# microsoft/DiskANN

Hardware: NVIDIA H100
Metric: QPS @ recall@10>=0.95, 1Mx128 f32 L2 (Vamana R=64 greedy search, batch 10K) (higher is better)
Workload: dtype f32

## Files before the change

diskann_b200/csrc/dab_common.cuh:

```cuda
#pragma once

#include <cuda_fp16.h>
#include <cuda_runtime.h>

#include <atomic>
#include <cstdarg>
#include <cstdint>
#include <cstdio>
#include <cstring>

#include "../../include/diskann_b200.h"

struct dab_index;

namespace dab {

constexpr uint32_t kNoId = 0xFFFFFFFFu;

char* error_buffer();
int fail(int code, const char* fmt, ...);
extern std::atomic<uint64_t> g_launches;
void comm_release(struct ::dab_index* idx);
void tc_release(struct ::dab_index* idx);
void search_slots_release(struct ::dab_index* idx);

#define DAB_CUDA(expr)                                                                        \
    do {                                                                                      \
        cudaError_t _e = (expr);                                                              \
        if (_e != cudaSuccess)                                                                \
            return ::dab::fail(_e == cudaErrorMemoryAllocation ? DAB_ERR_OUT_OF_MEMORY         \
                                                               : DAB_ERR_CUDA,               \
                               "%s failed: %s (%s:%d)", #expr, cudaGetErrorString(_e),        \
                               __FILE__, __LINE__);                                           \
    } while (0)

#define DAB_LAUNCHED() (::dab::g_launches.fetch_add(1, std::memory_order_relaxed))

inline size_t elem_size(int dtype) {
    switch (dtype) {
        case DAB_F32: return 4;
        case DAB_F16: return 2;
        default: return 1;
    }
}
inline size_t round_up(size_t x, size_t m) { return (x + m - 1) / m * m; }

struct Scratch {
    void* p = nullptr;
    size_t bytes = 0;
    bool pinned_host = false;
    int reserve(size_t n);
    void release();
};

struct Tuning {
    int test_visited_log2 = 0;
    bool test_pq_global_lut = false;
    void load();
};

}

struct dab_index {
    int dtype = 0, metric = 0;
    uint32_t dim = 0;
    uint64_t n_points = 0;
    uint32_t n_start = 0;
    uint32_t max_degree = 0;
    int device = 0;
    int sm_count = 132;

    cudaStream_t stream = nullptr;
    cudaStream_t own_stream = nullptr;

    uint8_t* d_vectors = nullptr;
    size_t row_stride = 0;
    uint32_t* d_adj = nullptr;
    uint32_t adj_stride = 0;
    bool vectors_ready = false, graph_ready = false;

    float* d_pivots = nullptr;
    uint32_t* d_offsets = nullptr;
    uint8_t* d_codes = nullptr;
    uint32_t pq_chunks = 0, pq_centers = 0;
    uint32_t pq_uniform_len = 0;
    bool pq_codes_ready = false;
    int sq_nbits = 0;
    float sq_scale = 0.0f, sq_shift_square_norm = 0.0f, sq_mean_norm = 0.0f;
    float* d_sq_shift = nullptr;
    uint8_t* d_sq_codes = nullptr;
    float* d_sq_comp = nullptr;
    uint32_t sq_row_bytes = 0, sq_stride = 0;
    bool sq_codes_ready = false;

    dab::Scratch s_queries, s_ids, s_out, s_out2, s_tables, s_counters, s_stats;
    dab::Scratch h_stage;
    dab::Scratch h_counters;
    void* slots[DAB_MAX_SLOTS] = {};

    uint32_t hint_l = 0, hint_beam = 0, hint_visited = 0;
    uint32_t pq_hint_l = 0, pq_hint_beam = 0, pq_hint_visited = 0; int pq_hint_mode = 0;
    uint32_t v3_overflow_l = 0, v3_overflow_beam = 0;
    float v3_overflow_frac = 0.0f;
    void* l2_window_ptr = nullptr;
    size_t l2_window_bytes = 0;
    cudaStream_t l2_window_stream = nullptr;

    uint64_t rec_truncated = 0;
    dab::Tuning tune;

    void* d_tc_base = nullptr;
    void* d_tc_coef = nullptr;
    uint64_t tc_version = 0, vectors_version = 1;

    void* nccl_comm = nullptr;
    int nccl_rank = 0, nccl_ranks = 0;

    uint64_t n_total() const { return n_points + n_start; }
};
```

diskann_b200/csrc/search_kernel.cu:

```cuda
#include "dab_common.cuh"
#include "distance_device.cuh"
#include "search_v2.cuh"
#include "search_v3.cuh"

#include <algorithm>
#include <cstdlib>

namespace dab {

constexpr int kSearchWarps = 4;
constexpr uint32_t kEmpty = 0xFFFFFFFFu;
constexpr uint32_t kVisitedFlag = 0x80000000u;
constexpr int kRowsInFlight = 4;

struct SearchParams {
    const uint8_t* vectors;
    size_t row_stride;
    const uint32_t* adj;
    uint32_t adj_stride;
    uint64_t n_points;
    uint32_t n_start;
    uint32_t dim;
    uint32_t max_degree;
    const void* queries;
// ... 185 lines not shown
                    else if (c0 == 64) word = w2;
                    else word = c0 + lane < p.adj_stride ? __ldg(row + c0 + lane) : kEmpty;
                    const uint32_t j = c0 + lane;
                    const bool valid = j >= 1 && j <= deg;
                    bool inserted = false;
                    if (valid) inserted = visited_insert(table, p.hcap_log2, word);
                    const bool isnew = inserted && word < n_total;
                    const unsigned mi = __ballot_sync(kFull, inserted);
                    const unsigned mn = __ballot_sync(kFull, isnew);
                    if (isnew) cid[ncand + __popc(mn & ((1u << lane) - 1u))] = word;
                    ncand += __popc(mn);
                    nvisited += __popc(mi);
                }
                if (nvisited + p.max_degree + 32 > hlimit) {
                    overflow = true;
                    break;
                }
            }
            if (overflow) break;
            __syncwarp();

            for (uint32_t c0 = 0; c0 < ncand; c0 += TEAMS * U) {
                float r[U];
                uint32_t cc[U];
                if constexpr (IS_INT) {
                    const uint8_t* rows[U];
#pragma unroll
                    for (int u = 0; u < U; ++u) {
                        cc[u] = c0 + u;
                        const uint32_t id = cid[min(cc[u], ncand - 1)];
                        rows[u] = p.vectors + (size_t)id * p.row_stride;
                    }
                    warp_int_multi<SIGNED, KIND, U>(qb, rows, dim, lane, qq, r);
                } else {
                    const TD* rows[U];
#pragma unroll
                    for (int u = 0; u < U; ++u) {
                        cc[u] = c0 + u * TEAMS + team;
                        const uint32_t id = cid[min(cc[u], ncand - 1)];
                        rows[u] = reinterpret_cast<const TD*>(p.vectors + (size_t)id * p.row_stride);
                    }
                    team_float_multi<NA, KIND, U>(qf, rows, dim, slot, r);
                }
#pragma unroll
                for (int u = 0; u < U; ++u)
                    if (slot == 0 && cc[u] < ncand) cd[cc[u]] = post_op<POST>(r[u]);
            }
            __syncwarp();

            for (uint32_t c = 0; c < ncand; ++c) queue_insert(qd, qi, p.cap, size, cursor, cid[c], cd[c], lane);
            cmps += ncand;
            hops += nb;
        }

        if (overflow) {
            if (lane == 0) {
                uint32_t o = atomicAdd(p.counters + 1, 1u);
                p.overflow_list[o] = qidx;
            }
            continue;
        }

        {
            const uint32_t n = min(p.cap, size);
            uint32_t count = 0;
            for (uint32_t b = 0; b < n && count < p.k; b += 32) {
                const uint32_t i = b + lane;
                uint32_t id = i < n ? (qi[i] & ~kVisitedFlag) : kEmpty;
                const bool keep = i < n && id < p.n_points;
                const unsigned m = __ballot_sync(kFull, keep);
                const uint32_t pos = count + __popc(m & ((1u << lane) - 1u));
                if (keep && pos < p.k) {
                    p.out_ids[(size_t)qidx * p.k + pos] = id;
                    p.out_dists[(size_t)qidx * p.k + pos] = qd[i];
                }
                count += __popc(m);
            }
            count = min(count, p.k);
            for (uint32_t i = count + lane; i < p.k; i += 32) {
                p.out_ids[(size_t)qidx * p.k + i] = kEmpty;
                p.out_dists[(size_t)qidx * p.k + i] = __int_as_float(0x7F800000);
            }
            if (lane == 0) {
                atomicMax(p.counters + 2, nvisited);
                if (p.out_counts) p.out_counts[qidx] = count;
                if (p.out_cmps) p.out_cmps[qidx] = cmps;
                if (p.out_hops) p.out_hops[qidx] = hops;
                if (p.rec_counts) {
                    p.rec_counts[qidx] = min(nrec, p.rec_cap);
                    if (nrec > p.rec_cap) atomicAdd(p.counters + 3, 1u);
                }
            }
        }
    }
}


constexpr int kV2WarpsHost = kV2Warps;

static uint32_t next_pow2_log2(uint64_t v) {
    uint32_t l = 0;
    while ((1ull << l) < v) ++l;
    return l;
}

static void pin_tables_in_l2(dab_index* idx, size_t bytes) {
    void* want = bytes ? idx->s_tables.p : nullptr;
    if (idx->l2_window_ptr == want && idx->l2_window_bytes == bytes && (bytes == 0 || idx->l2_window_stream == idx->stream)) return;
    cudaStreamAttrValue attr;
    memset(&attr, 0, sizeof(attr));
    if (bytes == 0) {
        attr.accessPolicyWindow.num_bytes = 0;
        attr.accessPolicyWindow.hitProp = cudaAccessPropertyNormal;
        attr.accessPolicyWindow.missProp = cudaAccessPropertyNormal;
        if (cudaStreamSetAttribute(idx->l2_window_stream, cudaStreamAttributeAccessPolicyWindow, &attr) != cudaSuccess) cudaGetLastError();
        idx->l2_window_ptr = nullptr;
        idx->l2_window_bytes = 0;
        return;
    }
    int max_persist = 0, max_window = 0;
    cudaDeviceGetAttribute(&max_persist, cudaDevAttrMaxPersistingL2CacheSize, idx->device);
    cudaDeviceGetAttribute(&max_window, cudaDevAttrMaxAccessPolicyWindowSize, idx->device);
    if (max_persist <= 0 || max_window <= 0) return;
    cudaDeviceSetLimit(cudaLimitPersistingL2CacheSize, (size_t)max_persist);
    attr.accessPolicyWindow.base_ptr = idx->s_tables.p;
    attr.accessPolicyWindow.num_bytes = std::min<size_t>(bytes, (size_t)max_window);
    attr.accessPolicyWindow.hitRatio = bytes <= (size_t)max_persist ? 1.0f : (float)((double)max_persist / (double)bytes);
    attr.accessPolicyWindow.hitProp = cudaAccessPropertyPersisting;
    attr.accessPolicyWindow.missProp = cudaAccessPropertyStreaming;
    if (cudaStreamSetAttribute(idx->stream, cudaStreamAttributeAccessPolicyWindow, &attr) != cudaSuccess) {
        cudaGetLastError();
        return;
    }
    idx->l2_window_ptr = idx->s_tables.p;
    idx->l2_window_bytes = bytes;
    idx->l2_window_stream = idx->stream;
}

template <typename K>
static int launch_one(K kern, const dab_index* idx, SearchParams& p, size_t smem_block, int& grid_out) {
    DAB_CUDA(cudaFuncSetAttribute(kern, cudaFuncAttributeMaxDynamicSharedMemorySize, (int)smem_block));
    int per_sm = 0;
    DAB_CUDA(cudaOccupancyMaxActiveBlocksPerMultiprocessor(&per_sm, kern, kSearchWarps * 32, smem_block));
    if (per_sm < 1) return fail(DAB_ERR_INVALID_ARGUMENT, "search kernel does not fit: %zu B shared memory per CTA", smem_block);
    grid_out = per_sm * idx->sm_count;
    return DAB_OK;
}

struct SearchJob {
    dab_index* idx = nullptr;
    cudaStream_t stream = nullptr;
    Scratch* tables = nullptr;
    Scratch* counters = nullptr;
    uint32_t* h_counters = nullptr;
    bool use_window = false;
    bool full_grid = false;

    uint32_t nq = 0, l_search = 0, beam = 0;
    bool recording = false;
    SearchParams p;
    SearchParamsV2 p2;
    SearchParamsV3 p3;
    void (*kern)(const SearchParams) = nullptr;
    size_t smem_block = 0;
    int grid = 0;
    bool use_v2 = false;
    V2Launch v2;
    V3Launch v3;
    uint64_t slots = 0;
    int stage = 1;
    int pass = 0;
    Scratch retry_list;
    uint32_t *d_counters = nullptr, *d_overflow = nullptr;

    int prepare(const void* d_queries, const uint32_t* d_query_rows, uint32_t nq_, uint32_t k, uint32_t l_search_, uint32_t beam_,
                uint32_t* d_ids, float* d_dists, uint32_t* d_counts, uint32_t* d_cmps, uint32_t* d_hops, uint32_t* rec_ids,
                float* rec_dists, uint32_t* rec_counts, uint32_t rec_cap);
    int launch();
    int finish();
    ~SearchJob() { retry_list.release(); }
};

int SearchJob::prepare(const void* d_queries, const uint32_t* d_query_rows, uint32_t nq_, uint32_t k, uint32_t l_search_,
                       uint32_t beam_, uint32_t* d_ids, float* d_dists, uint32_t* d_counts, uint32_t* d_cmps, uint32_t* d_hops,
                       uint32_t* rec_ids, float* rec_dists, uint32_t* rec_counts, uint32_t rec_cap) {
    nq = nq_, l_search = l_search_, beam = beam_;
    recording = rec_ids != nullptr;
    const bool is_int = idx->dtype == DAB_I8 || idx->dtype == DAB_U8;
    const MetricPlan plan = plan_for(idx->metric, is_int);

    memset(&p, 0, sizeof(p));
    p.vectors = idx->d_vectors;
    p.row_stride = idx->row_stride;
    p.adj = idx->d_adj;
    p.adj_stride = idx->adj_stride;
    p.n_points = idx->n_points;
    p.n_start = idx->n_start;
    p.dim = idx->dim;
    p.max_degree = idx->max_degree;
    p.queries = d_queries;
    p.query_rows = d_query_rows;
    p.k = k;
    p.cap = l_search + idx->n_start;
    p.beam = beam;
    p.out_ids = d_ids;
    p.out_dists = d_dists;
    p.out_counts = d_counts;
    p.out_cmps = d_cmps;
    p.out_hops = d_hops;
    p.rec_ids = rec_ids;
    p.rec_dists = rec_dists;
    p.rec_counts = rec_counts;
    p.rec_cap = rec_cap;

    size_t off = 0;
    const size_t qbytes = is_int ? round_up(idx->dim, 4) : (size_t)idx->dim * 4;
    off = round_up(qbytes, 16);
    p.off_qd = (uint32_t)off;
    off += round_up((size_t)p.cap * 4, 16);
    p.off_qi = (uint32_t)off;
    off += round_up((size_t)p.cap * 4, 16);
    const size_t ncand_max = (size_t)beam * idx->max_degree;
    p.off_cid = (uint32_t)off;
    off += round_up(ncand_max * 4, 16);
    p.off_cd = (uint32_t)off;
    off += round_up(ncand_max * 4, 16);
    p.off_beam = (uint32_t)off;
    off += round_up((size_t)beam * 4, 16);
    p.warp_smem = (uint32_t)off;
    smem_block = off * kSearchWarps;
    if (smem_block > 220 * 1024)
        return fail(DAB_ERR_INVALID_ARGUMENT, "search: L=%u, beam=%u, dim=%u need %zu B shared memory per CTA (> 220 KiB)",
                    l_search, beam, idx->dim, smem_block);

    int rc = DAB_OK;
#define PICK(TD, NA, K, P, II, SG)                               \
    do {                                                         \
        kern = search_kernel<TD, NA, K, P, II, SG>;              \
        rc = launch_one(kern, idx, p, smem_block, grid);         \
    } while (0)
#define PICK_FLOAT(TD)                                                                   \
    do {                                                                                 \
        if (plan.kind == KIND_L2) PICK(TD, 4, KIND_L2, POST_ID, false, false);            \
        else if (plan.kind == KIND_IP && plan.post == POST_NEG) PICK(TD, 4, KIND_IP, POST_NEG, false, false); \
        else if (plan.kind == KIND_IP) PICK(TD, 4, KIND_IP, POST_ONE_MINUS, false, false); \
        else PICK(TD, 2, KIND_COS, POST_ONE_MINUS, false, false);                         \
    } while (0)
#define PICK_INT(SG)                                                                     \
    do {                                                                                 \
        if (plan.kind == KIND_L2) PICK(uint8_t, 4, KIND_L2, POST_ID, true, SG);           \
        else if (plan.kind == KIND_IP) PICK(uint8_t, 4, KIND_IP, POST_NEG, true, SG);     \
        else PICK(uint8_t, 4, KIND_COS, POST_ONE_MINUS, true, SG);                        \
    } while (0)
    switch (idx->dtype) {
        case DAB_F32: PICK_FLOAT(float); break;
        case DAB_F16: PICK_FLOAT(__half); break;
        case DAB_I8: PICK_INT(true); break;
        default: PICK_INT(false); break;
    }
#undef PICK
#undef PICK_FLOAT
#undef PICK_INT
    if (rc) return rc;

    memset(&p2, 0, sizeof(p2));
    use_v2 = v2_prepare(idx, l_search, beam, full_grid, p2, v2) == 0;
    if (use_v2) {
        p2.vectors = p.vectors;
        p2.row_stride = p.row_stride;
        p2.adj = p.adj;
        p2.adj_stride = p.adj_stride;
        p2.n_points = p.n_points;
        p2.n_start = p.n_start;
        p2.dim = p.dim;
        p2.max_degree = p.max_degree;
        p2.queries = p.queries;
        p2.query_rows = p.query_rows;
        p2.k = p.k;
        p2.cap = p.cap;
        p2.beam = p.beam;
        p2.out_ids = p.out_ids;
        p2.out_dists = p.out_dists;
        p2.out_counts = p.out_counts;
        p2.out_cmps = p.out_cmps;
        p2.out_hops = p.out_hops;
        p2.rec_ids = p.rec_ids;
        p2.rec_dists = p.rec_dists;
        p2.rec_counts = p.rec_counts;
        p2.rec_cap = p.rec_cap;
        grid = v2.grid;
    }

    double est = 1.1 * idx->max_degree * 1.3 * (double)l_search;
    const bool hinted = idx->hint_visited > 0 && l_search <= idx->hint_l && beam <= idx->hint_beam;
    if (hinted) {
        const double seen = ((double)idx->hint_visited * 1.15 + idx->max_degree) / (use_v2 ? 0.875 : 0.75) + 8.0;
        if (seen < est) est = seen;
    }
    if (est > (double)idx->n_total() * 1.34) est = (double)idx->n_total() * 1.34;
    slots = std::max<uint64_t>(256, (uint64_t)est + 1);
    if (idx->tune.test_visited_log2) slots = 1ull << idx->tune.test_visited_log2;

    if ((rc = counters->reserve(16 + (size_t)nq * 4))) return rc;
    d_counters = (uint32_t*)counters->p;
    d_overflow = d_counters + 4;
    p.counters = d_counters;
    p.overflow_list = d_overflow;
    p.n_work = nq;
    p.query_list = nullptr;
    p2.counters = d_counters;
    p2.overflow_list = d_overflow;

    stage = 1;
    pass = 0;
    uint32_t need = 0;
    if (hinted) need = (uint32_t)std::min<double>((double)idx->hint_visited * 1.15, 4.0e9);
    if (idx->tune.test_visited_log2) need = (1u << idx->tune.test_visited_log2) / 2;
    const bool skip = idx->v3_overflow_l == l_search && idx->v3_overflow_beam == beam && idx->v3_overflow_frac > 0.25f;
    memset(&p3, 0, sizeof(p3));
    if (!skip && v3_prepare(idx, l_search, beam, need, p3, v3) == 0) {
        stage = 0;
        p3.vectors = p.vectors, p3.row_stride = p.row_stride, p3.adj = p.adj, p3.adj_stride = p.adj_stride;
        p3.n_points = p.n_points, p3.n_start = p.n_start, p3.dim = p.dim, p3.max_degree = p.max_degree;
        p3.queries = p.queries, p3.query_rows = p.query_rows, p3.query_list = nullptr, p3.n_work = nq;
        p3.k = p.k, p3.cap = p.cap, p3.beam = p.beam;
        p3.out_ids = p.out_ids, p3.out_dists = p.out_dists, p3.out_counts = p.out_counts;
        p3.out_cmps = p.out_cmps, p3.out_hops = p.out_hops;
        p3.rec_ids = p.rec_ids, p3.rec_dists = p.rec_dists, p3.rec_counts = p.rec_counts, p3.rec_cap = p.rec_cap;
        p3.counters = d_counters, p3.overflow_list = d_overflow;
    }
    return DAB_OK;
}

int SearchJob::launch() {
    DAB_CUDA(cudaMemsetAsync(d_counters, 0, 16, stream));
    if (stage == 0) {
        const uint64_t max_workers = (uint64_t)v3.grid * kV3Warps;
        const uint64_t rounds = (nq + max_workers - 1) / max_workers;
        const uint64_t need_warps = (nq + rounds - 1) / rounds;
        const int launch_grid = (int)((need_warps + kV3Warps - 1) / kV3Warps);
        v3.kern<<<launch_grid, kV3Warps * 32, v3.smem_block, stream>>>(p3);
    } else {
        const uint32_t warps = (uint32_t)grid * (use_v2 ? kV2WarpsHost : kSearchWarps);
        const uint32_t hlog = std::max<uint32_t>(use_v2 ? 8 : 10, next_pow2_log2(slots));
        const uint32_t n_buckets = (uint32_t)((slots + 7) / 8);
        const size_t words_per_warp = use_v2 ? (size_t)n_buckets * 8 : ((size_t)1 << hlog);
        int rc;
        if ((rc = tables->reserve((size_t)warps * words_per_warp * 4))) return rc;
        p.tables = (uint32_t*)tables->p;
        p.hcap_log2 = hlog;
        if (use_window) pin_tables_in_l2(idx, use_v2 ? 0 : (size_t)warps * words_per_warp * 4);
        if (use_v2) {
            const uint64_t max_warps = (uint64_t)grid * kV2WarpsHost;
            const uint64_t rounds = (p.n_work + max_warps - 1) / max_warps;
            const uint64_t need = (p.n_work + rounds - 1) / rounds;
            int launch_grid = (int)((need + kV2WarpsHost - 1) / kV2WarpsHost);
            if (full_grid) launch_grid = (int)std::min<uint64_t>((uint64_t)grid, ((uint64_t)p.n_work + kV2WarpsHost - 1) / kV2WarpsHost);
            p2.tables = p.tables;
            p2.n_buckets = n_buckets;
            p2.query_list = p.query_list;
            p2.n_work = p.n_work;
            v2.kern<<<launch_grid, kV2WarpsHost * 32, v2.smem_block, stream>>>(p2);
        } else {
            const int launch_grid = (int)std::min<uint64_t>((uint64_t)grid, ((uint64_t)p.n_work + kSearchWarps - 1) / kSearchWarps);
            kern<<<launch_grid, kSearchWarps * 32, smem_block, stream>>>(p);
        }
    }
    DAB_LAUNCHED();
    DAB_CUDA(cudaGetLastError());
    DAB_CUDA(cudaMemcpyAsync(h_counters, d_counters, 16, cudaMemcpyDeviceToHost, stream));
    return DAB_OK;
}

int SearchJob::finish() {
    for (;;) {
        DAB_CUDA(cudaStreamSynchronize(stream));
        idx->rec_truncated += h_counters[3];
        const uint32_t n_over = h_counters[1];
        if (!recording) {
            if (l_search != idx->hint_l || beam != idx->hint_beam) {
                idx->hint_l = l_search;
                idx->hint_beam = beam;
                idx->hint_visited = 0;
            }
            idx->hint_visited = std::max(idx->hint_visited, h_counters[2]);
            if (stage == 0) {
                idx->v3_overflow_l = l_search;
                idx->v3_overflow_beam = beam;
                idx->v3_overflow_frac = (float)n_over / (float)nq;
            }
        }
        if (n_over == 0) {
            retry_list.release();
            return DAB_OK;
        }
        Scratch next;
        int rc;
        if ((rc = next.reserve((size_t)n_over * 4))) return rc;
        DAB_CUDA(cudaMemcpyAsync(next.p, d_overflow, (size_t)n_over * 4, cudaMemcpyDeviceToDevice, stream));
        DAB_CUDA(cudaStreamSynchronize(stream));
        retry_list.release();
        retry_list = next;
        p.query_list = (const uint32_t*)retry_list.p;
        p.n_work = n_over;
        if (stage == 0) {
            stage = 1;
            pass = 0;
            if (!idx->tune.test_visited_log2)
                slots = std::max<uint64_t>(slots, std::min<uint64_t>((uint64_t)(1.1 * idx->max_degree * 1.3 * (double)l_search) + 1,
                                                                        (uint64_t)((double)idx->n_total() * 1.34) + 1));
        } else {
            if (++pass >= 6) {
                retry_list.release();
                return fail(DAB_ERR_VISITED_OVERFLOW, "search: visited set still overflowing after 6 passes");
            }
            slots *= 4;
            if (slots > 4 * idx->n_total() + 4096) slots = 2 * idx->n_total() + 2048;
        }
        if ((rc = launch())) return rc;
    }
}

static int check_search_args(const dab_index* idx, uint32_t k, uint32_t l_search, uint32_t beam) {
    if (!idx->vectors_ready || !idx->graph_ready) return fail(DAB_ERR_NOT_READY, "search: vectors and graph must be uploaded first");
    if (k == 0 || l_search == 0 || beam == 0) return fail(DAB_ERR_INVALID_ARGUMENT, "search: k, l_search and beam_width must be > 0");
    if (beam > 64) return fail(DAB_ERR_INVALID_ARGUMENT, "search: beam_width %u > 64", beam);
    return DAB_OK;
}

int run_search(dab_index* idx, const void* d_queries, const uint32_t* d_query_rows, uint32_t nq, uint32_t k,
               uint32_t l_search, uint32_t beam, uint32_t* d_ids, float* d_dists, uint32_t* d_counts, uint32_t* d_cmps,
               uint32_t* d_hops, uint32_t* rec_ids, float* rec_dists, uint32_t* rec_counts, uint32_t rec_cap) {
    int rc;
    if ((rc = check_search_args(idx, k, l_search, beam))) return rc;
    if (nq == 0) return DAB_OK;
    if ((rc = idx->h_counters.reserve(16))) return rc;
    SearchJob job;
    job.idx = idx;
    job.stream = idx->stream;
    job.tables = &idx->s_tables;
    job.counters = &idx->s_counters;
    job.h_counters = (uint32_t*)idx->h_counters.p;
    job.use_window = true;
    if ((rc = job.prepare(d_queries, d_query_rows, nq, k, l_search, beam, d_ids, d_dists, d_counts, d_cmps, d_hops, rec_ids,
                          rec_dists, rec_counts, rec_cap)))
        return rc;
    if ((rc = job.launch())) return rc;
    return job.finish();
}

struct AsyncHostOut {
    uint32_t* ids;
    float* dists;
    uint32_t *counts, *cmps, *hops;
    uint32_t nq, k;
};

struct SearchSlot {
    cudaStream_t stream = nullptr;
    Scratch tables, counters, queries, out, stats, h_counters;
    SearchJob* job = nullptr;
    AsyncHostOut host_out{};
    bool has_host_out = false;
};

void search_slots_release(dab_index* idx) {
    for (int i = 0; i < DAB_MAX_SLOTS; ++i) {
        SearchSlot* s = (SearchSlot*)idx->slots[i];
        if (!s) continue;
        if (s->stream) cudaStreamSynchronize(s->stream);
        delete s->job;
        s->tables.release(), s->counters.release(), s->queries.release(), s->out.release(), s->stats.release(), s->h_counters.release();
        if (s->stream) cudaStreamDestroy(s->stream);
        delete s;
        idx->slots[i] = nullptr;
    }
}

static int slot_of(dab_index* idx, uint32_t slot, SearchSlot** out) {
    if (slot >= DAB_MAX_SLOTS) return fail(DAB_ERR_INVALID_ARGUMENT, "search: slot %u out of range (DAB_MAX_SLOTS = %d)", slot, DAB_MAX_SLOTS);
    SearchSlot* s = (SearchSlot*)idx->slots[slot];
    if (!s) {
        s = new SearchSlot();
        s->h_counters.pinned_host = true;
        if (cudaStreamCreateWithFlags(&s->stream, cudaStreamNonBlocking) != cudaSuccess) {
            delete s;
            return fail(DAB_ERR_CUDA, "search: cannot create the stream of slot %u", slot);
        }
        idx->slots[slot] = s;
    }
    *out = s;
    return DAB_OK;
}

static int slot_launch(dab_index* idx, SearchSlot* s, const void* d_queries, uint32_t nq, uint32_t k, uint32_t l_search, uint32_t beam,
                       uint32_t* d_ids, float* d_dists, uint32_t* d_counts, uint32_t* d_cmps, uint32_t* d_hops) {
    int rc;
    if ((rc = s->h_counters.reserve(16))) return rc;
    SearchJob* job = new SearchJob();
    job->idx = idx;
    job->stream = s->stream;
    job->tables = &s->tables;
    job->counters = &s->counters;
    job->h_counters = (uint32_t*)s->h_counters.p;
    job->full_grid = true;
    if ((rc = job->prepare(d_queries, nullptr, nq, k, l_search, beam, d_ids, d_dists, d_counts, d_cmps, d_hops, nullptr, nullptr,
                           nullptr, 0)) ||
        (rc = job->launch())) {
        delete job;
        return rc;
    }
    s->job = job;
    return DAB_OK;
}

}

using namespace dab;

extern "C" {

int dab_search_batch_device(dab_index* idx, const void* d_queries, uint32_t nq, uint32_t k, uint32_t l_search,
                            uint32_t beam_width, uint32_t* d_out_ids, float* d_out_dists, uint32_t* d_out_counts,
                            uint32_t* d_out_cmps, uint32_t* d_out_hops) {
    if (!idx) return fail(DAB_ERR_INVALID_ARGUMENT, "dab_search_batch: idx is NULL");
    if (nq && (!d_queries || !d_out_ids || !d_out_dists)) return fail(DAB_ERR_INVALID_ARGUMENT, "dab_search_batch: NULL argument");
    DAB_CUDA(cudaSetDevice(idx->device));
    return run_search(idx, d_queries, nullptr, nq, k, l_search, beam_width, d_out_ids, d_out_dists, d_out_counts,
                      d_out_cmps, d_out_hops, nullptr, nullptr, nullptr, 0);
}

int dab_search_batch(dab_index* idx, const void* queries, uint32_t nq, uint32_t k, uint32_t l_search,
                     uint32_t beam_width, uint32_t* out_ids, float* out_dists, uint32_t* out_counts,
                     uint32_t* out_cmps, uint32_t* out_hops) {
    if (!idx) return fail(DAB_ERR_INVALID_ARGUMENT, "dab_search_batch: idx is NULL");
    if (nq == 0) return DAB_OK;
    if (!queries || !out_ids || !out_dists) return fail(DAB_ERR_INVALID_ARGUMENT, "dab_search_batch: NULL argument");
    if (k == 0) return fail(DAB_ERR_INVALID_ARGUMENT, "dab_search_batch: k must be > 0");
    DAB_CUDA(cudaSetDevice(idx->device));
    const size_t qbytes = (size_t)nq * idx->dim * elem_size(idx->dtype);
    const size_t rbytes = (size_t)nq * k * 4;
    int rc;
    if ((rc = idx->s_queries.reserve(qbytes))) return rc;
    if ((rc = idx->s_out.reserve(2 * rbytes))) return rc;
    if ((rc = idx->s_stats.reserve((size_t)nq * 12))) return rc;
    uint32_t* d_ids = (uint32_t*)idx->s_out.p;
    float* d_dists = (float*)((uint8_t*)idx->s_out.p + rbytes);
    uint32_t* d_counts = (uint32_t*)idx->s_stats.p;
    uint32_t* d_cmps = d_counts + nq;
    uint32_t* d_hops = d_cmps + nq;
    DAB_CUDA(cudaMemcpyAsync(idx->s_queries.p, queries, qbytes, cudaMemcpyHostToDevice, idx->stream));
    if ((rc = run_search(idx, idx->s_queries.p, nullptr, nq, k, l_search, beam_width, d_ids, d_dists, d_counts, d_cmps,
                         d_hops, nullptr, nullptr, nullptr, 0)))
        return rc;
    DAB_CUDA(cudaMemcpyAsync(out_ids, d_ids, rbytes, cudaMemcpyDeviceToHost, idx->stream));
    DAB_CUDA(cudaMemcpyAsync(out_dists, d_dists, rbytes, cudaMemcpyDeviceToHost, idx->stream));
    if (out_counts) DAB_CUDA(cudaMemcpyAsync(out_counts, d_counts, (size_t)nq * 4, cudaMemcpyDeviceToHost, idx->stream));
    if (out_cmps) DAB_CUDA(cudaMemcpyAsync(out_cmps, d_cmps, (size_t)nq * 4, cudaMemcpyDeviceToHost, idx->stream));
    if (out_hops) DAB_CUDA(cudaMemcpyAsync(out_hops, d_hops, (size_t)nq * 4, cudaMemcpyDeviceToHost, idx->stream));
    DAB_CUDA(cudaStreamSynchronize(idx->stream));
    return DAB_OK;
}

static int queue_result_copies(SearchSlot* s, const AsyncHostOut& o) {
    const size_t rbytes = (size_t)o.nq * o.k * 4;
    uint32_t* d_ids = (uint32_t*)s->out.p;
    float* d_dists = (float*)((uint8_t*)s->out.p + rbytes);
    uint32_t* d_counts = (uint32_t*)s->stats.p;
    DAB_CUDA(cudaMemcpyAsync(o.ids, d_ids, rbytes, cudaMemcpyDeviceToHost, s->stream));
    DAB_CUDA(cudaMemcpyAsync(o.dists, d_dists, rbytes, cudaMemcpyDeviceToHost, s->stream));
    if (o.counts) DAB_CUDA(cudaMemcpyAsync(o.counts, d_counts, (size_t)o.nq * 4, cudaMemcpyDeviceToHost, s->stream));
    if (o.cmps) DAB_CUDA(cudaMemcpyAsync(o.cmps, d_counts + o.nq, (size_t)o.nq * 4, cudaMemcpyDeviceToHost, s->stream));
    if (o.hops) DAB_CUDA(cudaMemcpyAsync(o.hops, d_counts + 2 * (size_t)o.nq, (size_t)o.nq * 4, cudaMemcpyDeviceToHost, s->stream));
    return DAB_OK;
}

int dab_search_batch_async(dab_index* idx, uint32_t slot, const void* queries, uint32_t nq, uint32_t k, uint32_t l_search,
                           uint32_t beam_width, uint32_t* out_ids, float* out_dists, uint32_t* out_counts, uint32_t* out_cmps,
                           uint32_t* out_hops) {
    if (!idx) return fail(DAB_ERR_INVALID_ARGUMENT, "dab_search_batch_async: idx is NULL");
    if (nq && (!queries || !out_ids || !out_dists)) return fail(DAB_ERR_INVALID_ARGUMENT, "dab_search_batch_async: NULL argument");
    int rc;
    if ((rc = check_search_args(idx, k, l_search, beam_width))) return rc;
    DAB_CUDA(cudaSetDevice(idx->device));
    SearchSlot* s = nullptr;
    if ((rc = slot_of(idx, slot, &s))) return rc;
    if (s->job) return fail(DAB_ERR_INVALID_ARGUMENT, "dab_search_batch_async: slot %u still has a batch in flight (call dab_wait)", slot);
    if (nq == 0) return DAB_OK;
    const size_t qbytes = (size_t)nq * idx->dim * elem_size(idx->dtype);
    const size_t rbytes = (size_t)nq * k * 4;
    if ((rc = s->queries.reserve(qbytes))) return rc;
    if ((rc = s->out.reserve(2 * rbytes))) return rc;
    if ((rc = s->stats.reserve((size_t)nq * 12))) return rc;
    uint32_t* d_ids = (uint32_t*)s->out.p;
    float* d_dists = (float*)((uint8_t*)s->out.p + rbytes);
    uint32_t* d_counts = (uint32_t*)s->stats.p;
    DAB_CUDA(cudaMemcpyAsync(s->queries.p, queries, qbytes, cudaMemcpyHostToDevice, s->stream));
    if ((rc = slot_launch(idx, s, s->queries.p, nq, k, l_search, beam_width, d_ids, d_dists, d_counts, d_counts + nq, d_counts + 2 * (size_t)nq)))
        return rc;
    s->host_out = AsyncHostOut{out_ids, out_dists, out_counts, out_cmps, out_hops, nq, k};
    s->has_host_out = true;
    return queue_result_copies(s, s->host_out);
}

int dab_search_batch_device_async(dab_index* idx, uint32_t slot, const void* d_queries, uint32_t nq, uint32_t k, uint32_t l_search,
                                  uint32_t beam_width, uint32_t* d_out_ids, float* d_out_dists, uint32_t* d_out_counts,
                                  uint32_t* d_out_cmps, uint32_t* d_out_hops) {
    if (!idx) return fail(DAB_ERR_INVALID_ARGUMENT, "dab_search_batch_device_async: idx is NULL");
    if (nq && (!d_queries || !d_out_ids || !d_out_dists)) return fail(DAB_ERR_INVALID_ARGUMENT, "dab_search_batch_device_async: NULL argument");
    int rc;
    if ((rc = check_search_args(idx, k, l_search, beam_width))) return rc;
    DAB_CUDA(cudaSetDevice(idx->device));
    SearchSlot* s = nullptr;
    if ((rc = slot_of(idx, slot, &s))) return rc;
    if (s->job) return fail(DAB_ERR_INVALID_ARGUMENT, "dab_search_batch_device_async: slot %u still has a batch in flight (call dab_wait)", slot);
    if (nq == 0) return DAB_OK;
    s->has_host_out = false;
    return slot_launch(idx, s, d_queries, nq, k, l_search, beam_width, d_out_ids, d_out_dists, d_out_counts, d_out_cmps, d_out_hops);
}

int dab_wait(dab_index* idx, uint32_t slot) {
    if (!idx) return fail(DAB_ERR_INVALID_ARGUMENT, "dab_wait: idx is NULL");
    if (slot >= DAB_MAX_SLOTS) return fail(DAB_ERR_INVALID_ARGUMENT, "dab_wait: slot %u out of range (DAB_MAX_SLOTS = %d)", slot, DAB_MAX_SLOTS);
    SearchSlot* s = (SearchSlot*)idx->slots[slot];
    if (!s || !s->job) return DAB_OK;
    DAB_CUDA(cudaSetDevice(idx->device));
    SearchJob* job = s->job;
    s->job = nullptr;
    DAB_CUDA(cudaStreamSynchronize(s->stream));
    const bool overflowed = job->h_counters[1] != 0;
    int rc = job->finish();
    delete job;
    if (rc) return rc;
    if (overflowed && s->has_host_out) {
        if ((rc = queue_result_copies(s, s->host_out))) return rc;
        DAB_CUDA(cudaStreamSynchronize(s->stream));
    }
    return DAB_OK;
}

}
```

diskann_b200/csrc/search_kernel_v2.cu:

```cuda
#include "dab_common.cuh"
#include "distance_device.cuh"
#include "search_common.cuh"
#include "search_v2.cuh"

#include <algorithm>
#include <cstdlib>
#include <type_traits>

namespace dab {

constexpr int kGroup = 8;
constexpr int kV2MinCtas = 21;
__device__ __forceinline__ uint32_t smem_u32(const void* p) { return (uint32_t)__cvta_generic_to_shared(p); }

__device__ __forceinline__ void prefetch_l2(const void* p) { asm volatile("prefetch.global.L2 [%0];" ::"l"(p)); }

template <int M>
__device__ __forceinline__ void bfly8(float (&v)[kGroup], int lane, int bit) {
    const bool up = (lane & bit) != 0;
#pragma unroll
    for (int i = 0; i < M / 2; ++i) {
        const float keep = up ? v[M / 2 + i] : v[i];
        const float send = up ? v[i] : v[M / 2 + i];
        v[i] = __fadd_rn(keep, __shfl_xor_sync(kFull, send, bit));
    }
}

template <typename TD, int KIND>
__device__ __forceinline__ float group_distance(const float* __restrict__ q, const uint8_t* __restrict__ rows,
                                                uint32_t row_slot, int dim, int lane) {
    const int full8 = dim & ~7, rem = dim & 7;
    float v[kGroup];
#pragma unroll
    for (int g = 0; g < kGroup; ++g) v[g] = 0.0f;
    for (int e = lane; e < full8; e += 32) {
        const float x = q[e];
#pragma unroll
        for (int g = 0; g < kGroup; ++g) {
            const float y = to_f32(reinterpret_cast<const TD*>(rows + (size_t)g * row_slot)[e]);
            if (KIND == KIND_L2) {
                const float c = __fsub_rn(x, y);
                v[g] = __fmaf_rn(c, c, v[g]);
            } else {
                v[g] = __fmaf_rn(x, y, v[g]);
            }
        }
    }
    bfly8<8>(v, lane, 8);
    bfly8<4>(v, lane, 16);
    if (rem) {
        const int hi = (((lane >> 4) & 1) << 1) | (((lane >> 3) & 1) << 2);
        const int l = lane & 7;
#pragma unroll
        for (int i = 0; i < 2; ++i) {
            const int g = i | hi;
            const float x = l < rem ? q[full8 + l] : 0.0f;
            const float y = l < rem ? to_f32(reinterpret_cast<const TD*>(rows + (size_t)g * row_slot)[full8 + l]) : 0.0f;
            if (KIND == KIND_L2) {
                const float c = __fsub_rn(x, y);
                v[i] = __fmaf_rn(c, c, v[i]);
            } else {
                v[i] = __fmaf_rn(x, y, v[i]);
            }
        }
    }
    bfly8<2>(v, lane, 4);
    float a = v[0];
    a = __fadd_rn(a, __shfl_xor_sync(kFull, a, 2));
    a = __fadd_rn(a, __shfl_xor_sync(kFull, a, 1));
    return a;
}

template <typename T>
struct V2Int {
    static constexpr bool value = false, is_signed = false;
};
template <>
struct V2Int<int8_t> {
    static constexpr bool value = true, is_signed = true;
};
template <>
struct V2Int<uint8_t> {
    static constexpr bool value = true, is_signed = false;
};

template <bool SIGNED, int KIND>
__device__ __forceinline__ void group_distance_int(const uint8_t* __restrict__ q, const uint8_t* __restrict__ rows, uint32_t row_slot, int dim,
                                                   int lane, int qq, float (&out)[kGroup]) {
    int xy[kGroup], yy[kGroup];
#pragma unroll
    for (int g = 0; g < kGroup; ++g) xy[g] = yy[g] = 0;
    const int nwords = dim >> 2;
    for (int w = lane; w < nwords; w += 32) {
        const int x = reinterpret_cast<const int*>(q)[w];
#pragma unroll
        for (int g = 0; g < kGroup; ++g) {
            const int y = reinterpret_cast<const int*>(rows + (size_t)g * row_slot)[w];
            xy[g] = dp4<SIGNED>(x, y, xy[g]);
            if (KIND != KIND_IP) yy[g] = dp4<SIGNED>(y, y, yy[g]);
        }
    }
    const int tail = dim & 3;
    if (lane < tail) {
        const int i = (nwords << 2) + lane;
        const int x = byte_at<SIGNED>(q, i);
#pragma unroll
        for (int g = 0; g < kGroup; ++g) {
            const int y = byte_at<SIGNED>(rows + (size_t)g * row_slot, i);
            xy[g] += x * y;
            if (KIND != KIND_IP) yy[g] += y * y;
        }
    }
#pragma unroll
    for (int g = 0; g < kGroup; ++g) {
        const int sxy = __reduce_add_sync(kFull, xy[g]);
        if (KIND == KIND_IP) {
            out[g] = (float)sxy;
        } else {
            const int syy = __reduce_add_sync(kFull, yy[g]);
            if (KIND == KIND_L2) out[g] = (float)(int)((unsigned)qq + (unsigned)syy - 2u * (unsigned)sxy);
            else out[g] = cosine_finish((float)qq, (float)syy, (float)sxy);
        }
    }
}

__device__ __forceinline__ void clear_global_table(uint32_t* table, uint32_t nbk, int lane) {
#pragma unroll 1
    for (uint32_t i = lane; i < nbk; i += 32) store_empty_bucket(table + (size_t)i * 8);
    __syncwarp();
}
__device__ __forceinline__ bool global_table_insert(uint32_t* table, uint32_t nbk, uint32_t id) {
    uint32_t bs[8];
    const uint32_t b = bucket_of(id, nbk);
    load_bucket(table + (size_t)b * 8, bs);
    return bucket_insert(table, nbk, b, bs, id);
}

template <typename TD, int KIND, int POST, int QT, bool L1>
__global__ void __launch_bounds__(kV2Warps * 32, kV2MinCtas) search_kernel_v2(const SearchParamsV2 p) {
    extern __shared__ __align__(128) uint8_t smem[];
    const int lane = threadIdx.x & 31, wib = threadIdx.x >> 5;
    uint8_t* base = smem + (size_t)wib * p.warp_smem;
    float* qf = reinterpret_cast<float*>(base + p.off_q);
    float* qd = reinterpret_cast<float*>(base + p.off_qd);
    uint32_t* qi = reinterpret_cast<uint32_t*>(base + p.off_qi);
    uint32_t* cid = reinterpret_cast<uint32_t*>(base + p.off_cid);
    float* cd = reinterpret_cast<float*>(base + p.off_cd);
    uint32_t* beam_ids = reinterpret_cast<uint32_t*>(base + p.off_beam);
    uint8_t* rows = base + p.off_rows;
    const uint32_t rows_a = smem_u32(rows);
    uint32_t* adjbuf = reinterpret_cast<uint32_t*>(base + p.off_adj);
    const uint32_t adjbuf_a = smem_u32(adjbuf);

    uint32_t* t1 = reinterpret_cast<uint32_t*>(base + p.off_t1);
    const uint32_t nb1 = p.t1_buckets;
    const Tag16Map tmap{p.tag_kmask, nb1, p.tag_magic, p.tag_shift};

    const uint32_t warp_slot = blockIdx.x * kV2Warps + wib;
    const uint32_t nbk = p.n_buckets;
    uint32_t* table = p.tables + (size_t)warp_slot * nbk * 8;
    const uint32_t hlimit = nbk * 7;
    const uint64_t n_total = p.n_points + p.n_start;
    const int dim = (int)p.dim;
    uint64_t row_policy;
    asm volatile("createpolicy.fractional.L2::evict_first.b64 %0, 1.0;" : "=l"(row_policy));

    for (;;) {
        uint32_t w = 0;
        if (lane == 0) w = atomicAdd(p.counters, 1u);
        w = __shfl_sync(kFull, w, 0);
        if (w >= p.n_work) break;
        const uint32_t qidx = p.query_list ? p.query_list[w] : w;

        __syncwarp();
        {
            const TD* s = p.query_rows ? reinterpret_cast<const TD*>(p.vectors + (size_t)p.query_rows[qidx] * p.row_stride)
                                       : reinterpret_cast<const TD*>(p.queries) + (size_t)qidx * dim;
            if constexpr (V2Int<TD>::value) {
                uint8_t* qb = reinterpret_cast<uint8_t*>(qf);
                const int qbytes = (dim + 3) & ~3;
                for (int e = lane; e < qbytes; e += 32) qb[e] = e < dim ? reinterpret_cast<const uint8_t*>(s)[e] : 0;
            } else {
                for (int e = lane; e < dim; e += 32) qf[e] = to_f32(s[e]);
            }
            if constexpr (L1) {
                const uint4 e4 = make_uint4(kEmptyV2, kEmptyV2, kEmptyV2, kEmptyV2);
                for (uint32_t i = lane; i < nb1 * 2; i += 32) reinterpret_cast<uint4*>(t1)[i] = e4;
            } else {
                for (uint32_t i = lane; i < nbk; i += 32) store_empty_bucket(table + (size_t)i * 8);
            }
        }
        __syncwarp();
        int qq = 0;
        if constexpr (V2Int<TD>::value) {
            if (KIND != KIND_IP) qq = warp_int_self<V2Int<TD>::is_signed>(reinterpret_cast<const uint8_t*>(qf), dim, lane);
        }

        uint32_t size = 0, cursor_lo = 0, cmps = 0, hops = 0, nvisited = 0, nrec = 0;
        uint32_t n1 = 0;
        bool closed = false;
        bool l2_used = false;
        uint32_t pred = kEmptyV2;
        bool overflow = false;

        auto visit_l1 = [&](uint32_t id, bool ok) -> bool {
            bool ins = false, need = false;
            if (ok) {
                uint32_t b1, tg;
                tag16_of(id, tmap, b1, tg);
                const int r = tag16_probe(t1, nb1, b1, tg, !closed);
                ins = r == 1;
                need = r == 2;
            }
            n1 += __popc(__ballot_sync(kFull, ins));
            if (__any_sync(kFull, need)) {
                if (!l2_used) {
                    clear_global_table(table, nbk, lane);
                    l2_used = true;
                }
                bool ins2 = false;
                if (need) ins2 = global_table_insert(table, nbk, id);
                nvisited += __popc(__ballot_sync(kFull, ins2));
                ins |= ins2;
            }
            return ins;
        };


        auto distances = [&](uint32_t c0, uint32_t n) {
            const uint32_t sub = (uint32_t)lane >> 3, nsub = 4, off0 = ((uint32_t)lane & 7u) * 16u, offs = 128;
            auto copy16 = [&](uint32_t dst, const uint8_t* src) {
                asm volatile("cp.async.cg.shared.global.L2::cache_hint [%0], [%1], 16, %2;" ::"r"(dst), "l"(src), "l"(row_policy) : "memory");
            };
            auto issue = [&](uint32_t lo, uint32_t hi) {
                if (p.row_bytes == 4 * offs) {
                    for (uint32_t j = lo + sub; j < hi; j += nsub) {
                        const uint8_t* src = p.vectors + (size_t)cid[c0 + j] * p.row_stride + off0;
                        const uint32_t dst = rows_a + j * p.row_slot + off0;
#pragma unroll
                        for (uint32_t k = 0; k < 4; ++k) copy16(dst + k * offs, src + k * offs);
                    }
                } else {
                    for (uint32_t j = lo + sub; j < hi; j += nsub) {
                        const uint8_t* src = p.vectors + (size_t)cid[c0 + j] * p.row_stride;
                        const uint32_t dst = rows_a + j * p.row_slot;
                        for (uint32_t off = off0; off < p.row_bytes; off += offs) copy16(dst + off, src + off);
                    }
                }
                asm volatile("cp.async.commit_group;" ::: "memory");
            };
            auto compute = [&](uint32_t g0) {
                if constexpr (V2Int<TD>::value) {
                    float vals[kGroup];
                    group_distance_int<V2Int<TD>::is_signed, KIND>(reinterpret_cast<const uint8_t*>(qf), rows + (size_t)g0 * p.row_slot,
                                                                  p.row_slot, dim, lane, qq, vals);
#pragma unroll
                    for (int u = 0; u < kGroup; ++u)
                        if (lane == u && g0 + u < n) cd[c0 + g0 + u] = post_op<POST>(vals[u]);
                } else {
                    const float r = group_distance<TD, KIND>(qf, rows + (size_t)g0 * p.row_slot, p.row_slot, dim, lane);
                    const uint32_t u = (((lane >> 3) & 1) << 2) | (((lane >> 4) & 1) << 1) | ((lane >> 2) & 1);
                    if ((lane & 3) == 0 && g0 + u < n) cd[c0 + g0 + u] = post_op<POST>(r);
                }
            };
            issue(0, n);
            asm volatile("cp.async.wait_group 0;" ::: "memory");
            __syncwarp();
            for (uint32_t g0 = 0; g0 < n; g0 += kGroup) compute(g0);
            __syncwarp();
        };

        for (uint32_t s0 = 0; s0 < p.n_start; s0 += 32) {
            const uint32_t n = min(32u, p.n_start - s0);
            if constexpr (L1) {
                const uint32_t id = (uint32_t)p.n_points + s0 + lane;
                if ((uint32_t)lane < n) cid[lane] = id;
                visit_l1(id, (uint32_t)lane < n);
            } else if ((uint32_t)lane < n) {
                const uint32_t id = (uint32_t)p.n_points + s0 + lane;
                cid[lane] = id;
                uint32_t bs[8];
                const uint32_t b = bucket_of(id, nbk);
                load_bucket(table + (size_t)b * 8, bs);
                bucket_insert(table, nbk, b, bs, id);
            }
            __syncwarp();
            for (uint32_t c0 = 0; c0 < n; c0 += p.stage_rows) distances(c0, min(p.stage_rows, n - c0));
            merge_round<QT>(qd, qi, p.cap, size, cursor_lo, cid, cd, 0, n, lane);
            if constexpr (!L1) nvisited += n;
            cmps += n;
        }

        for (;;) {
            const uint32_t lim = min(p.cap, size);
            uint32_t nb = 0;
            while (nb < p.beam) {
                const uint32_t idx = first_unvisited(qi, cursor_lo, lim, lane);
                if (idx >= lim) break;
                const uint32_t id = qi[idx];
                __syncwarp();
                if (lane == 0) {
                    qi[idx] = id | kFlagV2;
                    beam_ids[nb] = id;
                    if (p.rec_ids && nrec < p.rec_cap) {
                        p.rec_ids[(size_t)qidx * p.rec_cap + nrec] = id;
                        p.rec_dists[(size_t)qidx * p.rec_cap + nrec] = qd[idx];
                    }
                }
                cursor_lo = idx + 1;
                ++nrec;
                ++nb;
                __syncwarp();
            }
            if (nb == 0) break;

            uint32_t ncand = 0;
            for (uint32_t b = 0; b < nb; ++b) {
                const uint32_t node = beam_ids[b];
                const uint32_t* row = p.adj + (size_t)node * p.adj_stride;
                uint32_t wd[3];
                if (b == 0 && p.adj_words) {
                    asm volatile("cp.async.wait_group 0;" ::: "memory");
                    __syncwarp();
                }
                if (b == 0 && node == pred) {
                    wd[0] = adjbuf[lane];
                    wd[1] = 32 + lane < p.adj_words ? adjbuf[32 + lane] : kEmptyV2;
                    wd[2] = 64 + lane < p.adj_words ? adjbuf[64 + lane] : kEmptyV2;
                    __syncwarp();
                } else {
                    wd[0] = __ldg(row + lane);
                    wd[1] = 32 + lane < p.adj_stride ? __ldg(row + 32 + lane) : kEmptyV2;
                    wd[2] = 64 + lane < p.adj_stride ? __ldg(row + 64 + lane) : kEmptyV2;
                }
                if (b == 0) {
                    const uint32_t nxt = first_unvisited(qi, cursor_lo, lim, lane);
                    pred = kEmptyV2;
                    if (nxt < lim) {
                        const uint32_t nid = qi[nxt] & ~kFlagV2;
                        const uint32_t* nrow = p.adj + (size_t)nid * p.adj_stride;
                        if (p.adj_words) {
                            pred = nid;
                            if ((uint32_t)lane * 4 < p.adj_words)
                                asm volatile("cp.async.cg.shared.global [%0], [%1], 16;" ::"r"(adjbuf_a + lane * 16), "l"(nrow + lane * 4)
                                             : "memory");
                            asm volatile("cp.async.commit_group;" ::: "memory");
                        } else if (lane < 3) {
                            prefetch_l2(nrow + lane * 32);
                        }
                    }
                }
                const uint32_t deg = min(__shfl_sync(kFull, wd[0], 0), p.max_degree);
                if constexpr (L1) {
#pragma unroll 1
                    for (uint32_t c0 = 0; c0 <= deg; c0 += 32) {
                        const uint32_t j = c0 + lane;
                        uint32_t word = c0 == 0 ? wd[0] : (c0 == 32 ? wd[1] : wd[2]);
                        if (c0 >= 96) word = j < p.adj_stride ? __ldg(row + j) : kEmptyV2;
                        const bool ins = visit_l1(word, j >= 1 && j <= deg);
                        const bool isnew = ins && word < n_total;
                        const unsigned mn = __ballot_sync(kFull, isnew);
                        if (isnew) cid[ncand + __popc(mn & ((1u << lane) - 1u))] = word;
                        ncand += __popc(mn);
                    }
                    if (!closed && n1 + p.max_degree > p.t1_limit) closed = true;
                } else {
                    bool valid[3];
                    uint32_t bk[3];
                    uint32_t bs[3][8];
#pragma unroll
                    for (int c = 0; c < 3; ++c) {
                        const uint32_t j = c * 32 + lane;
                        valid[c] = j >= 1 && j <= deg;
                        bk[c] = bucket_of(wd[c], nbk);
                        if (valid[c]) load_bucket(table + (size_t)bk[c] * 8, bs[c]);
                    }
#pragma unroll
                    for (int c = 0; c < 3; ++c) {
                        bool inserted = false;
                        if (valid[c]) inserted = bucket_insert(table, nbk, bk[c], bs[c], wd[c]);
                        const bool isnew = inserted && wd[c] < n_total;
                        const unsigned mi = __ballot_sync(kFull, inserted);
                        const unsigned mn = __ballot_sync(kFull, isnew);
                        if (isnew) cid[ncand + __popc(mn & ((1u << lane) - 1u))] = wd[c];
                        ncand += __popc(mn);
// ... 182 lines not shown
```

Measured before the change: 4.284 million.

## Reorder queries by nearest pivot for cache locality; drop evict-first hint when L1 set

Adds a pre-pass that assigns each query to its nearest of 64 sampled dataset pivots, then radix-sorts queries by pivot id. The search kernels consume the resulting query_list, so queries processed at the same time share graph regions and vector rows stay hot in L2. The pass runs only when the batch exceeds the worker count on full-grid launches, and it adds a small kernel plus a sort per batch. Separately, the v2 kernel skips the L2 evict_first policy when the L1 template variant is used.

```diff
diff --git a/diskann_b200/csrc/dab_common.cuh b/diskann_b200/csrc/dab_common.cuh
--- a/diskann_b200/csrc/dab_common.cuh
+++ b/diskann_b200/csrc/dab_common.cuh
@@ -59,6 +59,9 @@
     void load();
 };
 
+int order_queries(const struct ::dab_index* idx, cudaStream_t stream, const void* d_queries, const uint32_t* d_query_rows, uint32_t nq,
+                  Scratch& buf, const uint32_t** order);
+
 }
 
 struct dab_index {
diff --git a/diskann_b200/csrc/query_order.cu b/diskann_b200/csrc/query_order.cu
--- /dev/null
+++ b/diskann_b200/csrc/query_order.cu
@@ -0,0 +1,136 @@
+#include "dab_common.cuh"
+#include "distance_device.cuh"
+
+#include <cub/device/device_radix_sort.cuh>
+
+namespace dab {
+
+constexpr int kOrderPivots = 64;
+constexpr int kOrderPivotBits = 6;
+constexpr int kOrderThreads = kOrderPivots;
+constexpr int kOrderQueries = 32;
+constexpr int kOrderChunk = 64;
+
+__device__ __forceinline__ float widen(float v) { return v; }
+__device__ __forceinline__ float widen(__half v) { return __half2float(v); }
+__device__ __forceinline__ float widen(int8_t v) { return (float)v; }
+__device__ __forceinline__ float widen(uint8_t v) { return (float)v; }
+
+template <typename T, bool L2>
+__global__ void __launch_bounds__(kOrderThreads, 2) pivot_key_kernel(const uint8_t* __restrict__ vectors, size_t row_stride,
+                                                                  uint64_t n_points, const void* __restrict__ queries,
+                                                                  const uint32_t* __restrict__ query_rows, uint32_t nq, uint32_t dim,
+                                                                  uint32_t* __restrict__ keys, uint32_t* __restrict__ vals) {
+    __shared__ __align__(16) float qs[kOrderChunk][kOrderQueries];
+    __shared__ float best_d[kOrderThreads / 32][kOrderQueries];
+    __shared__ uint32_t best_i[kOrderThreads / 32][kOrderQueries];
+    const uint32_t q0 = blockIdx.x * kOrderQueries;
+    const uint32_t nqb = min((uint32_t)kOrderQueries, nq - q0);
+    const uint32_t piv = threadIdx.x;
+    const T* prow = reinterpret_cast<const T*>(vectors + (size_t)(n_points * piv / kOrderPivots) * row_stride);
+    float acc[kOrderQueries];
+#pragma unroll
+    for (int j = 0; j < kOrderQueries; ++j) acc[j] = 0.0f;
+
+    for (uint32_t e0 = 0; e0 < dim; e0 += kOrderChunk) {
+        const uint32_t ne = min((uint32_t)kOrderChunk, dim - e0);
+        __syncthreads();
+        for (uint32_t i = threadIdx.x; i < kOrderChunk * kOrderQueries; i += kOrderThreads) {
+            const uint32_t j = i / kOrderChunk, e = i % kOrderChunk;
+            float v = 0.0f;
+            if (j < nqb && e < ne) {
+                const uint32_t q = q0 + j;
+                const T* src = query_rows ? reinterpret_cast<const T*>(vectors + (size_t)query_rows[q] * row_stride)
+                                          : reinterpret_cast<const T*>(queries) + (size_t)q * dim;
+                v = widen(src[e0 + e]);
+            }
+            qs[e][j] = v;
+        }
+        __syncthreads();
+        for (uint32_t e = 0; e < ne; ++e) {
+            const float y = widen(prow[e0 + e]);
+#pragma unroll
+            for (int j = 0; j < kOrderQueries; j += 4) {
+                const float4 x = *reinterpret_cast<const float4*>(&qs[e][j]);
+                if (L2) {
+                    acc[j] = fmaf(x.x - y, x.x - y, acc[j]);
+                    acc[j + 1] = fmaf(x.y - y, x.y - y, acc[j + 1]);
+                    acc[j + 2] = fmaf(x.z - y, x.z - y, acc[j + 2]);
+                    acc[j + 3] = fmaf(x.w - y, x.w - y, acc[j + 3]);
+                } else {
+                    acc[j] = fmaf(x.x, y, acc[j]);
+                    acc[j + 1] = fmaf(x.y, y, acc[j + 1]);
+                    acc[j + 2] = fmaf(x.z, y, acc[j + 2]);
+                    acc[j + 3] = fmaf(x.w, y, acc[j + 3]);
+                }
+            }
+        }
+    }
+
+    const int lane = threadIdx.x & 31, warp = threadIdx.x >> 5;
+#pragma unroll
+    for (int j = 0; j < kOrderQueries; ++j) {
+        float d = L2 ? acc[j] : -acc[j];
+        uint32_t id = piv;
+#pragma unroll
+        for (int m = 16; m >= 1; m >>= 1) {
+            const float od = __shfl_xor_sync(kFull, d, m);
+            const uint32_t oi = __shfl_xor_sync(kFull, id, m);
+            if (od < d || (od == d && oi < id)) d = od, id = oi;
+        }
+        if (lane == 0) best_d[warp][j] = d, best_i[warp][j] = id;
+    }
+    __syncthreads();
+    if (threadIdx.x < nqb) {
+        const uint32_t j = threadIdx.x;
+        float d = best_d[0][j];
+        uint32_t id = best_i[0][j];
+        for (int w = 1; w < kOrderThreads / 32; ++w)
+            if (best_d[w][j] < d) d = best_d[w][j], id = best_i[w][j];
+        keys[q0 + j] = id;
+        vals[q0 + j] = q0 + j;
+    }
+}
+
+int order_queries(const dab_index* idx, cudaStream_t stream, const void* d_queries, const uint32_t* d_query_rows, uint32_t nq,
+                  Scratch& buf, const uint32_t** order) {
+    size_t tmp_bytes = 0;
+    cub::DeviceRadixSort::SortPairs(nullptr, tmp_bytes, (const uint32_t*)nullptr, (uint32_t*)nullptr, (const uint32_t*)nullptr,
+                                    (uint32_t*)nullptr, (int)nq, 0, kOrderPivotBits, stream);
+    const size_t off = round_up(tmp_bytes, 256);
+    int rc;
+    if ((rc = buf.reserve(off + (size_t)nq * 16))) return rc;
+    uint32_t* keys = (uint32_t*)((uint8_t*)buf.p + off);
+    uint32_t* vals = keys + nq;
+    uint32_t* keys_sorted = vals + nq;
+    uint32_t* vals_sorted = keys_sorted + nq;
+
+    const bool l2 = plan_for(idx->metric, idx->dtype == DAB_I8 || idx->dtype == DAB_U8).kind == KIND_L2;
+    const int grid = (int)((nq + kOrderQueries - 1) / kOrderQueries);
+#define KEYS(T, L)                                                                                                                  \
+    pivot_key_kernel<T, L><<<grid, kOrderThreads, 0, stream>>>(idx->d_vectors, idx->row_stride, idx->n_points, d_queries, d_query_rows, \
+                                                               nq, idx->dim, keys, vals)
+#define KEYS_T(T)              \
+    do {                       \
+        if (l2) KEYS(T, true); \
+        else KEYS(T, false);   \
+    } while (0)
+    switch (idx->dtype) {
+        case DAB_F32: KEYS_T(float); break;
+        case DAB_F16: KEYS_T(__half); break;
+        case DAB_I8: KEYS_T(int8_t); break;
+        default: KEYS_T(uint8_t); break;
+    }
+#undef KEYS_T
+#undef KEYS
+    DAB_LAUNCHED();
+    DAB_CUDA(cudaGetLastError());
+    const cudaError_t e = cub::DeviceRadixSort::SortPairs(buf.p, tmp_bytes, keys, keys_sorted, vals, vals_sorted, (int)nq, 0,
+                                                          kOrderPivotBits, stream);
+    if (e != cudaSuccess) return fail(DAB_ERR_CUDA, "search: radix sort of the query order failed: %s", cudaGetErrorString(e));
+    DAB_LAUNCHED();
+    *order = vals_sorted;
+    return DAB_OK;
+}
+
+}
diff --git a/diskann_b200/csrc/search_kernel.cu b/diskann_b200/csrc/search_kernel.cu
--- a/diskann_b200/csrc/search_kernel.cu
+++ b/diskann_b200/csrc/search_kernel.cu
@@ -361,6 +361,7 @@
     cudaStream_t stream = nullptr;
     Scratch* tables = nullptr;
     Scratch* counters = nullptr;
+    Scratch* order = nullptr;
     uint32_t* h_counters = nullptr;
     bool use_window = false;
     bool full_grid = false;
@@ -537,6 +538,14 @@
         p3.out_cmps = p.out_cmps, p3.out_hops = p.out_hops;
         p3.rec_ids = p.rec_ids, p3.rec_dists = p.rec_dists, p3.rec_counts = p.rec_counts, p3.rec_cap = p.rec_cap;
         p3.counters = d_counters, p3.overflow_list = d_overflow;
+    }
+
+    const uint64_t workers = stage == 0 ? (uint64_t)v3.grid * kV3Warps : (uint64_t)grid * (use_v2 ? kV2WarpsHost : kSearchWarps);
+    if (full_grid && nq > workers) {
+        const uint32_t* list = nullptr;
+        if ((rc = order_queries(idx, stream, d_queries, d_query_rows, nq, *order, &list))) return rc;
+        p.query_list = list;
+        p3.query_list = list;
     }
     return DAB_OK;
 }
@@ -667,7 +676,7 @@
 
 struct SearchSlot {
     cudaStream_t stream = nullptr;
-    Scratch tables, counters, queries, out, stats, h_counters;
+    Scratch tables, counters, order, queries, out, stats, h_counters;
     SearchJob* job = nullptr;
     AsyncHostOut host_out{};
     bool has_host_out = false;
@@ -679,7 +688,7 @@
         if (!s) continue;
         if (s->stream) cudaStreamSynchronize(s->stream);
         delete s->job;
-        s->tables.release(), s->counters.release(), s->queries.release(), s->out.release(), s->stats.release(), s->h_counters.release();
+        s->tables.release(), s->counters.release(), s->order.release(), s->queries.release(), s->out.release(), s->stats.release(), s->h_counters.release();
         if (s->stream) cudaStreamDestroy(s->stream);
         delete s;
         idx->slots[i] = nullptr;
@@ -711,6 +720,7 @@
     job->stream = s->stream;
     job->tables = &s->tables;
     job->counters = &s->counters;
+    job->order = &s->order;
     job->h_counters = (uint32_t*)s->h_counters.p;
     job->full_grid = true;
     if ((rc = job->prepare(d_queries, nullptr, nq, k, l_search, beam, d_ids, d_dists, d_counts, d_cmps, d_hops, nullptr, nullptr,
diff --git a/diskann_b200/csrc/search_kernel_v2.cu b/diskann_b200/csrc/search_kernel_v2.cu
--- a/diskann_b200/csrc/search_kernel_v2.cu
+++ b/diskann_b200/csrc/search_kernel_v2.cu
@@ -162,8 +162,8 @@
     const uint32_t hlimit = nbk * 7;
     const uint64_t n_total = p.n_points + p.n_start;
     const int dim = (int)p.dim;
-    uint64_t row_policy;
-    asm volatile("createpolicy.fractional.L2::evict_first.b64 %0, 1.0;" : "=l"(row_policy));
+    uint64_t row_policy = 0;
+    if constexpr (!L1) asm volatile("createpolicy.fractional.L2::evict_first.b64 %0, 1.0;" : "=l"(row_policy));
 
     for (;;) {
         uint32_t w = 0;
@@ -230,7 +230,11 @@
         auto distances = [&](uint32_t c0, uint32_t n) {
             const uint32_t sub = (uint32_t)lane >> 3, nsub = 4, off0 = ((uint32_t)lane & 7u) * 16u, offs = 128;
             auto copy16 = [&](uint32_t dst, const uint8_t* src) {
-                asm volatile("cp.async.cg.shared.global.L2::cache_hint [%0], [%1], 16, %2;" ::"r"(dst), "l"(src), "l"(row_policy) : "memory");
+                if constexpr (L1)
+                    asm volatile("cp.async.cg.shared.global [%0], [%1], 16;" ::"r"(dst), "l"(src) : "memory");
+                else
+                    asm volatile("cp.async.cg.shared.global.L2::cache_hint [%0], [%1], 16, %2;" ::"r"(dst), "l"(src), "l"(row_policy)
+                                 : "memory");
             };
             auto issue = [&](uint32_t lo, uint32_t hi) {
                 if (p.row_bytes == 4 * offs) {
```

Measured after the change: 4.369 million, median of 6. 2.0% higher.
